# liuzhenboo/Stereo-Visual-Odometry

Measured on AMD Instinct MI355X. Metric: stereo frames/sec on KITTI-00 1241x376; LK-kernel achieved HBM GB/s vs peak, higher is better.
Workload: dtype u8; 1 GPU; S0 synthetic KITTI-like stereo sequence 1241x376 (config #2 stand-in), FAST+LK track_mode LK_stereof2f_pnp, batched frame pairs (256 per step, 4 distinct chunks cycled), frames resident in HBM for `value`; `m1` (--full) = host-resident frames, H2D included; pairs_ok_last_step=256, parallelism=1 GPU

## Files before the change

### include/svo_abi.h

```cpp
#ifndef SVO_ABI_H
#define SVO_ABI_H

#include <stdint.h>

#ifdef __cplusplus
extern "C" {
#endif

#define SVO_ABI_VERSION 9

#define SVO_OK                 0
#define SVO_ERR_ARG           -1
#define SVO_ERR_HIP           -2
#define SVO_ERR_NOMEM         -3
#define SVO_ERR_STATE         -4
#define SVO_FAIL_FEW_KEYPOINTS 1
#define SVO_FAIL_FEW_TRACKS    2
#define SVO_FAIL_INLIER_RATIO  3
#define SVO_FAIL_ROTATION_GATE 4
#define SVO_FAIL_TRANSL_GATE   5
#define SVO_FAIL_CAPACITY      6

#define SVO_MEM_HOST   0
#define SVO_MEM_DEVICE 1
// ... 23 lines not shown
    double  P1[12], P2[12];
    int32_t track_mode;
    int32_t orb_nfeatures;
    float   orb_scale_factor;
    int32_t orb_nlevels;
    int32_t orb_ini_th, orb_min_th;
    int32_t lk_accum;
    int32_t fast_keep_strongest;
} svo_config;

#define SVO_MODE_LK  0
#define SVO_MODE_ORB 1
#define SVO_LK_ACCUM_EXACT 0
#define SVO_LK_ACCUM_SSE2  1
#define SVO_LK_ACCUM_SIMD128 2
#define SVO_LK_ACCUM_SSE2_LEGACY 3

typedef struct {
    double rvec[3], tvec[3], R[9];
    int32_t n_inliers, ransac_iters, best_iter, lm_iters, ok, _pad;
} svo_pnp_result;

typedef struct {
    int32_t ok;
    int32_t fail_stage;
    int32_t n_prev_kps, n_cur_kps, n_tracked, n_inliers;
    int32_t ransac_iters, lm_iters;
    double  rvec[3], tvec[3], R[9];
    double  T_rel_inv[16];
    double  pose[16];
} svo_step_result;

int         svo_abi_version(void);
int         svo_config_bytes(void);
void        svo_default_config(svo_config *cfg, int width, int height);
int         svo_device_count(int *n);
int         svo_create(const svo_config *cfg, int device, svo_ctx **out);
void        svo_destroy(svo_ctx *ctx);
const char *svo_last_error(const svo_ctx *ctx);
int         svo_set_stream(svo_ctx *ctx, void *hip_stream);
int         svo_sync(svo_ctx *ctx);
int         svo_wait_stream(svo_ctx *ctx, void *hip_stream);
int         svo_signal_stream(svo_ctx *ctx, void *hip_stream);
int         svo_signal_stream_inputs(svo_ctx *ctx, void *hip_stream);
int         svo_num_levels(const svo_ctx *ctx);


int svo_fast_detect(svo_ctx *ctx, const uint8_t *img, int pitch, int mem, int threshold,
                    int nonmax, svo_keypoint *out, int cap, int *n_out);

int svo_build_pyramid(svo_ctx *ctx, int slot, const uint8_t *img, int pitch, int mem);
int svo_read_pyramid_level(svo_ctx *ctx, int slot, int level, uint8_t *out, int out_pitch, int mem,
                           int *w, int *h);

int svo_lk_track(svo_ctx *ctx, int slot_prev, int slot_next, const svo_pt2f *prev_pts, int n,
                 svo_pt2f *next_pts, uint8_t *status, int mem);

int svo_circular_match(svo_ctx *ctx, int slot_prevL, int slot_prevR, int slot_curL, int slot_curR,
                       const svo_pt2f *t1_left, int n, svo_pt2f *out_t1_left,
                       svo_pt2f *out_t1_right, svo_pt2f *out_t2_right, svo_pt2f *out_t2_left,
                       int *m_out, int mem);

int svo_triangulate(svo_ctx *ctx, const double P1[12], const double P2[12], const svo_pt2f *x1,
                    const svo_pt2f *x2, int n, svo_pt3f *out, int mem);

int svo_pnp_ransac(svo_ctx *ctx, const svo_pt3f *obj, const svo_pt2f *img, int n, const double K[9],
                   int iterations, float reproj_err, double confidence, svo_pnp_result *res,
                   uint8_t *inlier_mask, int mem);

int svo_orb_extract(svo_ctx *ctx, const uint8_t *img, int pitch, int mem, svo_keypoint *kps, uint8_t *desc,
                    int cap, int *n_out, int *per_level);
int svo_orb_read_level(svo_ctx *ctx, int level, uint8_t *out, int *w, int *h);
int svo_orb_read_candidates(svo_ctx *ctx, int level, float *out4, int cap, int *n_out);

int svo_match_hamming(svo_ctx *ctx, const uint8_t *query, int nq, const uint8_t *train, int nt, int32_t *train_idx,
                      float *distance, int mem);


int svo_add_frame(svo_ctx *ctx, const uint8_t *left, const uint8_t *right, int pitch, int mem,
                  svo_step_result *res);
int svo_reset(svo_ctx *ctx);
int svo_get_pose(svo_ctx *ctx, double pose[16]);
int svo_set_pose(svo_ctx *ctx, const double pose[16]);

int svo_track_batch(svo_ctx *ctx, const uint8_t *left_frames, const uint8_t *right_frames,
                    int pitch, int64_t frame_stride, int n_frames, const double *pose0,
                    svo_step_result *results, int results_mem);

int svo_set_overlap(svo_ctx *ctx, int on);
int svo_wait_results(svo_ctx *ctx);

int svo_host_alloc(svo_ctx *ctx, size_t bytes, void **out);
int svo_host_free(svo_ctx *ctx, void *p);
int svo_upload_frames(svo_ctx *ctx, int buf, const uint8_t *left_frames, const uint8_t *right_frames,
                      int pitch, int64_t frame_stride, int n_frames);
int svo_upload_frames_at(svo_ctx *ctx, int buf, int first_slot, const uint8_t *left_frames, const uint8_t *right_frames,
                         int pitch, int64_t frame_stride, int n_frames);
int svo_wait_upload(svo_ctx *ctx, int buf);
int svo_track_uploaded(svo_ctx *ctx, int buf, int n_frames, const double *pose0,
                       svo_step_result *results, int results_mem);
#define SVO_CONTINUE_CHAIN       1
#define SVO_CONTINUE_CARRY_FRAME 2
int svo_track_uploaded_async(svo_ctx *ctx, int buf, int n_frames, const double *pose0, int continue_chain);
int svo_collect_results(svo_ctx *ctx, svo_step_result *results, int n_pairs);
int svo_results_ready(svo_ctx *ctx, int *n_pairs);

// ... 133 lines not shown
```

### stereo-visual-odometry_amd/binding.py

```python
import ctypes as C
import os
import subprocess

import numpy as np

_HERE = os.path.dirname(os.path.abspath(__file__))
_LIB = None

MEM_HOST, MEM_DEVICE = 0, 1

KP_DTYPE = np.dtype([("x", "<f4"), ("y", "<f4"), ("size", "<f4"), ("angle", "<f4"),
                     ("response", "<f4"), ("octave", "<i4"), ("class_id", "<i4")])


class SvoError(RuntimeError):
    pass


class Config(C.Structure):
    _fields_ = [("width", C.c_int32), ("height", C.c_int32), ("max_keypoints", C.c_int32),
                ("max_batch", C.c_int32), ("num_slots", C.c_int32), ("fast_threshold", C.c_int32),
                ("num_features_tracking", C.c_int32), ("iterations", C.c_int32),
                ("reproj_err", C.c_float), ("confidence", C.c_float),
                ("feature_match_error", C.c_double), ("inlier_rate", C.c_double),
# ... 300 lines not shown
            return
        self.signal_stream(other)

    @property
    def num_levels(self):
        return self.lib.svo_num_levels(self.h)

    def set_overlap(self, on=True):
        self._check(self.lib.svo_set_overlap(self.h, int(on)))

    def wait_results(self):
        self._check(self.lib.svo_wait_results(self.h))

    def enable_timing(self, on=True):
        self._check(self.lib.svo_enable_timing(self.h, int(on)))

    def get_timing(self):
        names = (C.c_char_p * 64)()
        ms = (C.c_float * 64)()
        n = self.lib.svo_get_timing(self.h, names, ms, 64)
        return [(names[i].decode(), float(ms[i])) for i in range(n)]

    def _img(self, img, shape=None):
        shape = shape or (self.height, self.width)
        assert tuple(img.shape) == tuple(shape), (tuple(img.shape), shape)
        if isinstance(img, np.ndarray):
            assert img.dtype == np.uint8 and img.strides[1] == 1
            return C.c_void_p(img.ctypes.data), int(img.strides[0]), MEM_HOST
        assert img.element_size() == 1 and img.stride(1) == 1
        return C.c_void_p(img.data_ptr()), int(img.stride(0)), (MEM_DEVICE if img.is_cuda else MEM_HOST)

    def fast_detect(self, img, threshold=20, nonmax=True, cap=None):
        cap = cap or self.cfg.max_keypoints
        p, pitch, mem = self._img(img)
        out = np.zeros(cap, dtype=KP_DTYPE)
        n = C.c_int(0)
        self._check(self.lib.svo_fast_detect(self.h, p, pitch, mem, int(threshold), int(bool(nonmax)),
                                             C.c_void_p(out.ctypes.data), cap, C.byref(n)))
        return out[:n.value].copy()

    def build_pyramid(self, slot, img):
        p, pitch, mem = self._img(img)
        self._check(self.lib.svo_build_pyramid(self.h, int(slot), p, pitch, mem))

    def read_pyramid_level(self, slot, level):
        w, h = C.c_int(0), C.c_int(0)
        self._check(self.lib.svo_read_pyramid_level(self.h, slot, level, None, 0, MEM_HOST,
                                                    C.byref(w), C.byref(h)))
        out = np.zeros((h.value, w.value), np.uint8)
        self._check(self.lib.svo_read_pyramid_level(self.h, slot, level, C.c_void_p(out.ctypes.data),
                                                    w.value, MEM_HOST, C.byref(w), C.byref(h)))
        return out

    def lk_track(self, slot_prev, slot_next, pts):
        if isinstance(pts, np.ndarray):
            pts = np.ascontiguousarray(pts, np.float32).reshape(-1, 2)
            n = pts.shape[0]
            out = np.zeros((n, 2), np.float32)
            st = np.zeros(n, np.uint8)
        else:
            import torch
            n = pts.shape[0]
            out = torch.zeros((n, 2), dtype=torch.float32, device=pts.device)
            st = torch.zeros(n, dtype=torch.uint8, device=pts.device)
            self._order_in(st)
        pi, mem = _ptr(pts)
        po, _ = _ptr(out)
        ps, _ = _ptr(st)
        self._check(self.lib.svo_lk_track(self.h, slot_prev, slot_next, pi, n, po, ps, mem))
        if mem == MEM_DEVICE:
            self._order_out(st)
        return out, st

    def circular_match(self, slots, t1_left):
        if isinstance(t1_left, np.ndarray):
            t1_left = np.ascontiguousarray(t1_left, np.float32).reshape(-1, 2)
            n = t1_left.shape[0]
            outs = [np.zeros((max(n, 1), 2), np.float32) for _ in range(4)]
        else:
            import torch
            n = t1_left.shape[0]
            outs = [torch.zeros((max(n, 1), 2), dtype=torch.float32, device=t1_left.device) for _ in range(4)]
            self._order_in(outs[0])
        pi, mem = _ptr(t1_left)
        m = C.c_int(0)
        self._check(self.lib.svo_circular_match(self.h, *[int(s) for s in slots], pi, n,
                                                *[_ptr(o)[0] for o in outs], C.byref(m), mem))
        return [o[:m.value] for o in outs]

    def triangulate(self, P1, P2, x1, x2):
        P1 = np.ascontiguousarray(P1, np.float64).reshape(12)
        P2 = np.ascontiguousarray(P2, np.float64).reshape(12)
        if isinstance(x1, np.ndarray):
            x1 = np.ascontiguousarray(x1, np.float32).reshape(-1, 2)
            x2 = np.ascontiguousarray(x2, np.float32).reshape(-1, 2)
            out = np.zeros((x1.shape[0], 3), np.float32)
        else:
            import torch
            out = torch.zeros((x1.shape[0], 3), dtype=torch.float32, device=x1.device)
            self._order_in(out)
        p1, mem = _ptr(x1)
        p2, _ = _ptr(x2)
        self._check(self.lib.svo_triangulate(self.h, C.c_void_p(P1.ctypes.data), C.c_void_p(P2.ctypes.data),
                                             p1, p2, x1.shape[0], _ptr(out)[0], mem))
        if mem == MEM_DEVICE:
            self._order_out(out)
# ... 752 lines not shown
```

### stereo-visual-odometry_amd/csrc/pipeline.hip

```cpp
#include <cstring>
#include "abi_io.h"
#include "carry.h"

namespace svo {

void timing_mark(svo_ctx *ctx, const char *name)
{
    if (!ctx->timing) return;
    if (ctx->ev_used >= 16384) return;
    if (ctx->ev_used == ctx->ev_pool.size()) {
        hipEvent_t ev = nullptr;
        if (dev_event(ctx, &ev, hipEventDefault) != SVO_OK) return;
        ctx->ev_pool.push_back(ev);
    }
    hipEvent_t ev = ctx->ev_pool[ctx->ev_used++];
    (void)hipEventRecord(ev, ctx->stream);
    ctx->marks.emplace_back(name, ev);
}
static inline void mark(svo_ctx *ctx, const char *name) { timing_mark(ctx, name); }

static const char *kTMatch = "orb_match";
static const char *kT0 = "start", *kTPyr = "pyramid", *kTFast = "fast", *kTLk = "lk", *kTCompact = "compact",
                  *kTTri = "triangulate", *kTPnp = "pnp", *kTRefine = "refine", *kTFin = "finalize";

static int ingest_frames(svo_ctx *ctx, const uint8_t *L, const uint8_t *R, int pitch, int64_t frame_stride,
                         int f0, int n_new)
{
    if (ctx->cfg.track_mode == SVO_MODE_ORB) {
        const int rc = orb_extract_batch(ctx, L, R, pitch, frame_stride, 2 * f0, 2 * n_new, ctx->stream,  true);
        if (rc == SVO_OK && ctx->orbm_mode == SVO_ORB_MATCHER_GUIDED) return orbm_stereo_frames(ctx, 2 * f0, n_new, ctx->stream);
        return rc;
    }
    const PyrGeom &g = ctx->geom;
    PyrArgs p{};
    p.g = g; p.pitch = pitch; p.img_stride = frame_stride; p.slot_stride = g.slot_bytes;
    p.img = L; p.img2 = R; p.slots = ctx->bslots + (size_t)(2 * f0) * g.slot_bytes;
    launch_pyramid(p, 2 * n_new, ctx->stream);
    mark(ctx, kTPyr);
    if (ctx->lk_detector == SVO_DETECTOR_GFTT) {
        const int rc = gftt_detect_frames(ctx, L, pitch, frame_stride, f0, n_new);
        mark(ctx, kTFast);
        return rc;
    }
    FastArgs a{};
    a.img = L; a.pitch = pitch; a.img_stride = frame_stride;
    a.w = ctx->cfg.width; a.h = ctx->cfg.height; a.thr = ctx->cfg.fast_threshold; a.nms = 1;
    a.score = ctx->score + (size_t)f0 * ctx->score_stride; a.spitch = ctx->spitch; a.score_stride = ctx->score_stride;
    a.rowcount = ctx->rowcount + (size_t)f0 * ctx->rowcount_stride; a.rowcount_stride = ctx->rowcount_stride;
    a.kp_xy = ctx->kp_xy + (size_t)f0 * ctx->cfg.max_keypoints;
    a.kp_resp = ctx->kp_resp + (size_t)f0 * ctx->cfg.max_keypoints;
    a.kp_stride = ctx->cfg.max_keypoints;
    a.n_out = ctx->kp_n + f0; a.cap = ctx->cfg.max_keypoints;
    launch_fast(a, n_new, ctx->stream);
    if (ctx->bucket_keep > 0) {
        BucketArgs k{};
        k.kp_xy = a.kp_xy; k.kp_resp = a.kp_resp; k.kp_stride = a.kp_stride; k.n_out = a.n_out; k.cap = a.cap;
        k.w = a.w; k.h = a.h; k.cw = ctx->bucket_w; k.ch = ctx->bucket_h; k.per_cell = ctx->bucket_keep;
        k.cols = (a.w + k.cw - 1) / k.cw; k.ncells = k.cols * ((a.h + k.ch - 1) / k.ch);
        k.cells_stride = (int64_t)4 * k.ncells;
        k.cells = ctx->bucket_cells.base ? (int *)ctx->bucket_cells.base + (size_t)f0 * k.cells_stride : nullptr;
        launch_fast_buckets(k, n_new, ctx->stream);
    }
    launch_fast_keep_strongest(a, n_new, ctx->cfg.fast_keep_strongest, ctx->stream);
    mark(ctx, kTFast);
    return SVO_OK;
}

struct StreamStep { const int32_t *ids; const uint8_t *init; };
static int run_back(svo_ctx *ctx, int n_pairs, const double *pose0_host, svo_step_result *results_dev, bool triangulate_first = false,
                    const StreamStep *ss = nullptr);
static const char *kTGather = "stream_gather", *kTScatter = "stream_scatter";

static int stream_segments(svo_ctx *ctx, uint8_t *work[kMaxSeg], size_t bytes[kMaxSeg], int is_count[kMaxSeg])
{
    const size_t cap = (size_t)ctx->cfg.max_keypoints;
    if (ctx->cfg.track_mode == SVO_MODE_ORB) {
        const size_t kcap = (size_t)ctx->orb_kp_cap;
        work[0] = (uint8_t *)ctx->orb_kps;      bytes[0] = 2 * kcap * sizeof(svo_keypoint); is_count[0] = 0;
        work[1] = ctx->orb_desc;                bytes[1] = 2 * kcap * 32;                   is_count[1] = 0;
        work[2] = (uint8_t *)ctx->orb_n;        bytes[2] = 2 * sizeof(int);                 is_count[2] = 1;
        work[3] = (uint8_t *)ctx->orb_overflow; bytes[3] = 2 * sizeof(int);                 is_count[3] = 1;
        if (ctx->orbm_mode == SVO_ORB_MATCHER_GUIDED) {
            work[4] = ctx->orbm_frames;         bytes[4] = ctx->orbm_frame_bytes;           is_count[4] = 0;
            return 5;
        }
    } else {
        work[0] = ctx->bslots;                  bytes[0] = (size_t)2 * ctx->geom.slot_bytes; is_count[0] = 0;
        work[1] = (uint8_t *)ctx->kp_xy;        bytes[1] = cap * sizeof(float2);            is_count[1] = 0;
        work[2] = (uint8_t *)ctx->kp_resp;      bytes[2] = cap * sizeof(float);             is_count[2] = 0;
        work[3] = (uint8_t *)ctx->kp_n;         bytes[3] = sizeof(int);                     is_count[3] = 1;
// ... 482 lines not shown
```

### stereo-visual-odometry_amd/csrc/pyramid.hip

```cpp
#include "svo_device.h"
#include "svo_kernels.h"

namespace svo {

__device__ __forceinline__ const uint8_t *src_image(const PyrArgs &a, int b)
{
    if (a.img2) return ((b & 1) ? a.img2 : a.img) + (int64_t)(b >> 1) * a.img_stride;
    return a.img + (int64_t)b * a.img_stride;
}

__global__ __launch_bounds__(256) void pyr_copy0_kernel(PyrArgs a)
{
    const int b = blockIdx.z, y = blockIdx.y * blockDim.y + threadIdx.y;
    const int w = a.g.w[0];
    if (y >= a.g.h[0]) return;
    const uint8_t *src = src_image(a, b) + (int64_t)y * a.pitch;
    uint8_t *dst = a.slots + (int64_t)b * a.slot_stride + a.g.origin[0] + (int64_t)y * a.g.pitch[0];
    const int x = (blockIdx.x * blockDim.x + threadIdx.x) * 16;
    if (x >= w) return;
    if (x + 16 <= w && ((uintptr_t)(src + x) & 15) == 0) {
        *(uint4 *)(dst + x) = *(const uint4 *)(src + x);
    } else {
        for (int q = 0; q < 16 && x + q < w; q++) dst[x + q] = src[x + q];
    }
}

constexpr int kBorderRows = 16;
constexpr int kFrameRowsPerWg = 4, kSidePasses = 4;
__host__ __device__ inline int border_top_groups() { return 2 * kPad / kFrameRowsPerWg; }
__host__ __device__ inline int border_side_groups(int h) { return (h + kBorderRows * kSidePasses - 1) / (kBorderRows * kSidePasses); }
__global__ __launch_bounds__(256) void pyr_border_kernel(PyrArgs a, int l)
{
    const int b = blockIdx.y;
    const int w = a.g.w[l], h = a.g.h[l], pitch = a.g.pitch[l];
    uint8_t *lvl = a.slots + (int64_t)b * a.slot_stride + a.g.origin[l];
    if ((int)blockIdx.x < border_top_groups()) {
        for (int q = 0; q < kFrameRowsPerWg; q++) {
            const int gidx = blockIdx.x * kFrameRowsPerWg + q;
            const int py = gidx < kPad ? gidx - kPad : h + (gidx - kPad);
            const uint8_t *src = lvl + (int64_t)refl101(py, h) * pitch;
            uint8_t *dst = lvl + (int64_t)py * pitch;
            for (int px = ((int)threadIdx.x << 2) - kPad; px < w + kPad; px += 1024) {
                uint32_t v = 0;
                if (px >= 0 && px + 4 <= w) v = *(const uint32_t *)(src + px);
                else {
#pragma unroll
                    for (int k = 0; k < 4; k++) v |= (uint32_t)src[refl101(min(px + k, w + kPad - 1), w)] << (8 * k);
                }
                if (px + 4 <= w + kPad) *(uint32_t *)(dst + px) = v;
                else for (int k = 0; px + k < w + kPad; k++) dst[px + k] = (uint8_t)(v >> (8 * k));
            }
        }
        return;
    }
    const int sgroup = blockIdx.x - border_top_groups();
    if (w >= 2 * kPad) {
        static_assert(kBorderRows == 16 && kPad == 32, "256 threads = 16 rows x 16 dwords");
        typedef uint32_t u32_unaligned __attribute__((aligned(1)));
        const int k = threadIdx.x & 15, r = threadIdx.x >> 4;
        const int px = k < 8 ? -kPad + 4 * k : w + 4 * (k - 8);
        const int c0 = k < 8 ? kPad - 3 - 4 * k : w - 5 - 4 * (k - 8);
        for (int q = 0; q < kSidePasses; q++) {
            const int py = (sgroup * kSidePasses + q) * kBorderRows + r;
            if (py >= h) return;
            uint8_t *row = lvl + (int64_t)py * pitch;
            const uint32_t v = *(const u32_unaligned *)(row + c0);
            *(u32_unaligned *)(row + px) = __builtin_amdgcn_perm(0u, v, 0x00010203u);
        }
    } else {
        const int t = threadIdx.x & 63;
        const int px = t < kPad ? t - kPad : w + (t - kPad);
        const int sx = refl101(px, w);
        for (int q = 0; q < kSidePasses; q++)
            for (int r = threadIdx.x >> 6; r < kBorderRows; r += 4) {
                const int py = (sgroup * kSidePasses + q) * kBorderRows + r;
                if (py >= h) return;
                uint8_t *row = lvl + (int64_t)py * pitch;
                row[px] = row[sx];
            }
    }
}

__global__ __launch_bounds__(256) void pyr_down_kernel(PyrArgs a, int l)
{
    const int b = blockIdx.z, y = blockIdx.y * blockDim.y + threadIdx.y;
    const int w = a.g.w[l];
    if (y >= a.g.h[l]) return;
    const int sp = a.g.pitch[l - 1];
    uint8_t *slot = a.slots + (int64_t)b * a.slot_stride;
    const uint8_t *src = slot + a.g.origin[l - 1];
    uint8_t *dst = slot + a.g.origin[l] + (int64_t)y * a.g.pitch[l];
    const int x0 = (blockIdx.x * blockDim.x + threadIdx.x) * 4;
    if (x0 >= w) return;
    int acc[4] = {0, 0, 0, 0};
#pragma unroll
    for (int r = 0; r < 5; r++) {
        const uint32_t *row = (const uint32_t *)(src + (int64_t)(2 * y + r - 2) * sp + 2 * x0 - 4);
        const uint32_t d0 = row[0], d1 = row[1], d2 = row[2], d3 = row[3];
        int s[16];
#pragma unroll
        for (int j = 0; j < 4; j++) {
            s[j] = (d0 >> (8 * j)) & 255; s[4 + j] = (d1 >> (8 * j)) & 255;
            s[8 + j] = (d2 >> (8 * j)) & 255; s[12 + j] = (d3 >> (8 * j)) & 255;
        }
        const int wv = (r == 2) ? 6 : ((r == 1 || r == 3) ? 4 : 1);
#pragma unroll
        for (int q = 0; q < 4; q++) {
            const int c = 4 + 2 * q;
            const int hs = s[c] * 6 + (s[c - 1] + s[c + 1]) * 4 + s[c - 2] + s[c + 2];
            acc[q] += hs * wv;
        }
    }
    uint32_t out = 0;
#pragma unroll
    for (int q = 0; q < 4; q++) out |= (uint32_t)((acc[q] + 128) >> 8) << (8 * q);
    if (x0 + 4 <= w) *(uint32_t *)(dst + x0) = out;
    else for (int q = 0; x0 + q < w; q++) dst[x0 + q] = (uint8_t)(out >> (8 * q));
}

__global__ __launch_bounds__(256) void pyr_read_level_kernel(PyrGeom g, const uint8_t *slot, int l,
                                                              uint8_t *out, int out_pitch)
{
    int x = blockIdx.x * 256 + threadIdx.x, y = blockIdx.y;
    if (x >= g.w[l]) return;
    out[(int64_t)y * out_pitch + x] = slot[g.origin[l] + (int64_t)y * g.pitch[l] + x];
}

void launch_pyramid(const PyrArgs &a, int batch, hipStream_t st)
{
    dim3 blk(256, 1, 1);
    auto shape = [](int lanes_per_row, int rows, dim3 &grid, dim3 &block, int batch) {
        const int bx = lanes_per_row < 256 ? lanes_per_row : 256, by = 256 / bx;
        block = dim3(bx, by, 1);
        grid = dim3((lanes_per_row + bx - 1) / bx, (rows + by - 1) / by, batch);
    };
    {
        dim3 g, bk;
        shape((a.g.w[0] + 15) / 16, a.g.h[0], g, bk, batch);
        hipLaunchKernelGGL(pyr_copy0_kernel, g, bk, 0, st, a);
    }
    for (int l = 0; l < a.g.nlevels; l++) {
        if (l > 0) {
            dim3 g, bk;
            shape((a.g.w[l] + 3) / 4, a.g.h[l], g, bk, batch);
            hipLaunchKernelGGL(pyr_down_kernel, g, bk, 0, st, a, l);
        }
        dim3 gb(border_top_groups() + border_side_groups(a.g.h[l]), batch, 1);
        hipLaunchKernelGGL(pyr_border_kernel, gb, blk, 0, st, a, l);
    }
}

void launch_pyr_read_level(const PyrGeom &g, const uint8_t *slot, int l, uint8_t *out, int out_pitch,
                           hipStream_t st)
{
    dim3 grid((g.w[l] + 255) / 256, g.h[l], 1), blk(256, 1, 1);
    hipLaunchKernelGGL(pyr_read_level_kernel, grid, blk, 0, st, g, slot, l, out, out_pitch);
}

}
```

### stereo-visual-odometry_amd/csrc/svo_abi.hip

```cpp
#include <algorithm>
#include <cmath>
#include <cstdio>
#include <cstring>
#include <ctime>
#include <new>
#include <vector>
#include "abi_io.h"
#include "carry.h"
#include "fast_scratch.h"

using namespace svo;

namespace svo {
int dev_alloc_raw(svo_ctx *ctx, void **out, size_t bytes)
{
    *out = nullptr;
    if (bytes == 0) bytes = 1;
    if (ctx->arena.planning) {
        ctx->arena.plan.emplace_back(out, ctx->arena.planned);
        ctx->arena.planned += align_up(bytes, kDevAlign);
        return SVO_OK;
    }
    SVO_HIP(hipMalloc(out, bytes));
    ctx->arena.extra.push_back(*out);
    return SVO_OK;
}

int dev_defer(svo_ctx *ctx, std::function<int()> fn)
{
    if (!ctx->arena.planning) return fn();
    ctx->arena.after.push_back(std::move(fn));
    return SVO_OK;
}

static int dev_commit(svo_ctx *ctx)
{
    DevArena &a = ctx->arena;
    a.planning = false;
    SVO_HIP(hipMalloc((void **)&a.base, a.planned + 256));
    for (auto &e : a.plan) *e.first = a.base + e.second;
    a.plan.clear();
    for (auto &fn : a.after) { const int rc = fn(); if (rc != SVO_OK) return rc; }
    a.after.clear();
    return SVO_OK;
}

int dev_reserve(svo_ctx *ctx, DevScratch *s, size_t bytes)
{
    if (s->base && bytes <= s->bytes) return SVO_OK;
    uint8_t *grown = nullptr;
    SVO_HIP(hipMalloc((void **)&grown, bytes ? bytes : 1));
    uint8_t *old = s->base;
    if (!old) ctx->arena.scratch.push_back(s);
    s->base = grown; s->bytes = bytes;
    if (old) (void)hipFree(old);
    return SVO_OK;
}

int dev_event(svo_ctx *ctx, hipEvent_t *ev, unsigned flags)
{
    if (*ev) return SVO_OK;
    SVO_HIP(hipEventCreateWithFlags(ev, flags));
// ... 100 lines not shown
    DevArena &a = c->arena;
    for (hipEvent_t e : a.events) (void)hipEventDestroy(e);
    for (size_t k = a.streams.size(); k-- > 0;) (void)hipStreamDestroy(a.streams[k]);
    a.events.clear(); a.streams.clear();
}

static double now_ms()
{
    timespec ts;
    clock_gettime(CLOCK_MONOTONIC, &ts);
    return ts.tv_sec * 1e3 + ts.tv_nsec * 1e-6;
}
#define PHASE(name) do { if (timing_on) { const double t__ = now_ms(); fprintf(stderr, "[svo_create] %8.2f ms  %s\n", t__ - t_phase, name); t_phase = t__; } } while (0)

extern "C" int svo_create(const svo_config *cfg, int device, svo_ctx **out)
{
    if (!cfg || !out) return SVO_ERR_ARG;
    const bool timing_on = getenv("SVO_TIMING") != nullptr;
    double t_phase = now_ms();
    *out = nullptr;
    if (cfg->width < 32 || cfg->height < 32 || cfg->max_keypoints < 64 || cfg->max_batch < 1 ||
        cfg->num_slots < 4 || cfg->width > kMaxFrameSide || cfg->height > kMaxFrameSide)
        return SVO_ERR_ARG;
    if (cfg->lk_accum != SVO_LK_ACCUM_EXACT && cfg->lk_accum != SVO_LK_ACCUM_SSE2 && cfg->lk_accum != SVO_LK_ACCUM_SIMD128 &&
        cfg->lk_accum != SVO_LK_ACCUM_SSE2_LEGACY) {
        fprintf(stderr, "svo_create: lk_accum = %d is none of SVO_LK_ACCUM_EXACT / _SSE2 / _SIMD128 / _SSE2_LEGACY\n", cfg->lk_accum);
        return SVO_ERR_ARG;
    }
    if (cfg->fast_keep_strongest < 0) return SVO_ERR_ARG;
    if (cfg->num_features_tracking < 4) {
        fprintf(stderr, "svo_create: num_features_tracking = %d < 4 is not supported (cv::solvePnPRansac asserts npoints >= 4)\n",
                cfg->num_features_tracking);
        return SVO_ERR_ARG;
    }
    svo_ctx *ctx = new (std::nothrow) svo_ctx();
    if (!ctx) return SVO_ERR_NOMEM;
    ctx->cfg = *cfg;
    ctx->device = device;
    for (int i = 0; i < 16; i++) ctx->pose[i] = (i % 5 == 0) ? 1.0 : 0.0;
    int ndev = 0;
    if (hipGetDeviceCount(&ndev) != hipSuccess || ndev <= 0 || device < 0 || device >= ndev) {
        fprintf(stderr, "svo_create: no usable HIP device (count=%d, requested %d)\n", ndev, device);
        delete ctx;
        return SVO_ERR_HIP;
    }
    PHASE("hipGetDeviceCount (HIP runtime start)");
    auto fail = [&](int code) { free_all(ctx); delete ctx; return code; };
#define CK(call) do { if ((call) != 0) { fprintf(stderr, "svo_create: %s failed\n", #call); return fail(SVO_ERR_HIP); } } while (0)
    CK(hipSetDevice(device));
    CK(dev_stream(ctx, &ctx->own_stream));
    ctx->stream = ctx->own_stream;
    PHASE("hipSetDevice + stream");
    make_geom(cfg->width, cfg->height, &ctx->geom);

    const int w = cfg->width, h = cfg->height, cap = cfg->max_keypoints, B = cfg->max_batch;
    const int n_img = B + 1;
    ctx->n_img = n_img;
    const bool orb = cfg->track_mode == SVO_MODE_ORB;
    if (!orb && cfg->track_mode != SVO_MODE_LK) return fail(SVO_ERR_ARG);
    const int n_fast = orb ? 1 : n_img, B_lk = orb ? 1 : B;
    ctx->arena.planning = true;
#define DA(ptr, bytes) do { if (dev_alloc(ctx, &(ptr), (bytes)) != SVO_OK) return fail(SVO_ERR_HIP); } while (0)
    DA(ctx->slots, (size_t)cfg->num_slots * ctx->geom.slot_bytes);
    dev_defer(ctx, [ctx]() { SVO_HIP(hipMemsetAsync(ctx->slots, 0, (size_t)ctx->cfg.num_slots * ctx->geom.slot_bytes, ctx->stream)); return SVO_OK; });
    ctx->slot_built.assign(cfg->num_slots, 0);
    ctx->stage_pitch = align_up(w, 256);
    DA(ctx->stage_img, (size_t)ctx->stage_pitch * h * 2);
    ctx->spitch = fast_record_pitch(w);
    ctx->score_stride = (int64_t)ctx->spitch * h;
    DA(ctx->score, (size_t)ctx->score_stride * n_fast);
    ctx->rowcount_stride = fast_count_words(w, h);
    DA(ctx->rowcount, sizeof(int) * (size_t)ctx->rowcount_stride * n_fast);
    DA(ctx->kp_xy, sizeof(float2) * (size_t)cap * n_fast);
    DA(ctx->kp_resp, sizeof(float) * (size_t)cap * n_fast);
    DA(ctx->kp_n, sizeof(int) * (size_t)n_fast);
    DA(ctx->pts_in, sizeof(float2) * (size_t)cap * B_lk);
    for (int i = 0; i < 4; i++) {
        DA(ctx->pts_out[i], sizeof(float2) * (size_t)cap * B_lk);
        DA(ctx->status[i], (size_t)cap * B_lk);
        DA(ctx->cmp[i], sizeof(float2) * (size_t)cap * B);
    }
    DA(ctx->keep, (size_t)cap * B_lk);
    DA(ctx->m_out, sizeof(int) * (size_t)B);
    DA(ctx->X3, sizeof(float) * 3 * (size_t)cap * B);
    if (geom_workspace_bytes(*cfg, B, &ctx->pnp_ws_bytes) != SVO_OK) return fail(SVO_ERR_ARG);
    PHASE("plan + kernel attributes (code object load)");
    DA(ctx->pnp_ws, ctx->pnp_ws_bytes);
    dev_defer(ctx, [ctx]() { return geom_workspace_init(ctx); });
    DA(ctx->d_results, sizeof(svo_step_result) * (size_t)B);
    DA(ctx->bslots, orb ? 256 : (size_t)2 * n_img * ctx->geom.slot_bytes);
    DA(ctx->kp_n_snap, sizeof(int) * (size_t)(3 * n_img));
    if (B > 1) {
        const size_t per_cam = (size_t)ctx->stage_pitch * h * (size_t)(B + 1);
        for (int k = 0; k < 2; k++) {
            DA(ctx->fb[k], 2 * per_cam);
            DA(ctx->d_async[k], sizeof(svo_step_result) * (size_t)B);
        }
    }
    if (orb) {
        int rc = orb_alloc(ctx);
        if (rc != SVO_OK) { fprintf(stderr, "svo_create: %s\n", ctx->err.c_str()); return fail(rc); }
    }
#undef DA
    if (dev_commit(ctx) != SVO_OK) { fprintf(stderr, "svo_create: device memory (%zu MB): %s\n", ctx->arena.planned >> 20, ctx->err.c_str()); return fail(SVO_ERR_HIP); }
    PHASE("one device allocation + deferred initialisation");
    CK(hipHostMalloc(&ctx->h_stage, (size_t)ctx->stage_pitch * h * 2, hipHostMallocDefault));
// ... 146 lines not shown
    SVO_ARG(pitch >= ctx->cfg.width, "pitch < width");
    if (mem == SVO_MEM_DEVICE) { *dptr = img; *dpitch = pitch; return SVO_OK; }
    SVO_ARG(mem == SVO_MEM_HOST, "mem must be SVO_MEM_HOST or SVO_MEM_DEVICE");
    return svo::stage_host_image(ctx, img, pitch, stage_idx, dptr, dpitch);
}

extern "C" int svo_fast_detect(svo_ctx *ctx, const uint8_t *img, int pitch, int mem, int threshold,
                               int nonmax, svo_keypoint *out, int cap, int *n_out)
{
    if (!ctx) return SVO_ERR_ARG;
    SVO_ARG(out && n_out && cap >= 0, "null output");
    SVO_HIP(hipSetDevice(ctx->device));
    const uint8_t *d; int dp;
    int rc = resolve_image(ctx, img, pitch, mem, 0, &d, &dp);
    if (rc) return rc;
    FastArgs a{};
    a.img = d; a.pitch = dp; a.img_stride = 0;
    a.w = ctx->cfg.width; a.h = ctx->cfg.height;
    a.thr = threshold < 0 ? 0 : (threshold > 255 ? 255 : threshold);
    a.nms = nonmax != 0;
    a.score = ctx->score; a.spitch = ctx->spitch; a.score_stride = ctx->score_stride;
    a.rowcount = ctx->rowcount; a.rowcount_stride = ctx->rowcount_stride;
    a.kp_xy = ctx->kp_xy; a.kp_resp = ctx->kp_resp; a.kp_stride = ctx->cfg.max_keypoints;
    a.n_out = ctx->kp_n; a.cap = ctx->cfg.max_keypoints;
    launch_fast(a, 1, ctx->stream);
    SVO_HIP(hipGetLastError());
    int n;
    SVO_TRY(count_read(ctx, ctx->kp_n, &n));
    *n_out = n;
    if (n > ctx->cfg.max_keypoints) { ctx->err = "FAST: keypoints exceed max_keypoints"; return SVO_ERR_ARG; }
    if (n > cap) { ctx->err = "FAST: keypoints exceed caller capacity"; return SVO_ERR_ARG; }
    if (n == 0) return SVO_OK;
    float2 *h_xy;
    SVO_TRY(pinned_block(ctx, (sizeof(float2) + sizeof(float)) * (size_t)ctx->cfg.max_keypoints, &h_xy));
    float *h_r = (float *)(h_xy + ctx->cfg.max_keypoints);
    SVO_TRY(from_device(ctx, h_xy, (const float2 *)ctx->kp_xy, (size_t)n, SVO_MEM_HOST));
    SVO_TRY(from_device(ctx, h_r, (const float *)ctx->kp_resp, (size_t)n, SVO_MEM_HOST));
    SVO_TRY(io_done(ctx, SVO_MEM_HOST));
    format_keypoints(h_xy, h_r, n, out);
    return SVO_OK;
}

extern "C" int svo_build_pyramid(svo_ctx *ctx, int slot, const uint8_t *img, int pitch, int mem)
{
    if (!ctx) return SVO_ERR_ARG;
    SVO_ARG(slot >= 0 && slot < ctx->cfg.num_slots, "slot out of range");
    SVO_HIP(hipSetDevice(ctx->device));
    const uint8_t *d; int dp;
    int rc = resolve_image(ctx, img, pitch, mem, 0, &d, &dp);
    if (rc) return rc;
    PyrArgs a{};
    a.g = ctx->geom; a.img = d; a.pitch = dp; a.img_stride = 0;
    a.slots = ctx->slots + (size_t)slot * ctx->geom.slot_bytes; a.slot_stride = 0;
    launch_pyramid(a, 1, ctx->stream);
    SVO_HIP(hipGetLastError());
    if (mem == SVO_MEM_HOST) SVO_HIP(hipStreamSynchronize(ctx->stream));
    ctx->slot_built[slot] = 1;
    return SVO_OK;
}

extern "C" int svo_read_pyramid_level(svo_ctx *ctx, int slot, int level, uint8_t *out, int out_pitch,
                                      int mem, int *w, int *h)
{
    if (!ctx) return SVO_ERR_ARG;
    SVO_ARG(slot >= 0 && slot < ctx->cfg.num_slots, "slot out of range");
    SVO_ARG(level >= 0 && level < ctx->geom.nlevels, "level out of range");
    if (!ctx->slot_built[slot]) { ctx->err = "pyramid slot not built"; return SVO_ERR_STATE; }
    const int lw = ctx->geom.w[level], lh = ctx->geom.h[level];
    if (w) *w = lw;
    if (h) *h = lh;
    if (!out) return SVO_OK;
    SVO_ARG(out_pitch >= lw, "out_pitch < level width");
    SVO_HIP(hipSetDevice(ctx->device));
    const uint8_t *s = ctx->slots + (size_t)slot * ctx->geom.slot_bytes;
    if (mem == SVO_MEM_DEVICE) {
        launch_pyr_read_level(ctx->geom, s, level, out, out_pitch, ctx->stream);
        SVO_HIP(hipGetLastError());
        return SVO_OK;
    }
    SVO_HIP(hipMemcpy2DAsync(out, out_pitch, s + ctx->geom.origin[level], ctx->geom.pitch[level], lw, lh,
                             hipMemcpyDeviceToHost, ctx->stream));
    SVO_HIP(hipStreamSynchronize(ctx->stream));
    return SVO_OK;
}

static void fill_lk_common(svo_ctx *ctx, LkArgs &a, int n)
{
    a.g = ctx->geom;
    a.slot_stride = 0;
    a.pts_stride = 0;
    a.n_pts = nullptr; a.n_fixed = n; a.cap = n;
    a.match_err = ctx->cfg.feature_match_error;
    a.accum = ctx->cfg.lk_accum;
}

extern "C" int svo_lk_track(svo_ctx *ctx, int slot_prev, int slot_next, const svo_pt2f *prev_pts, int n,
                            svo_pt2f *next_pts, uint8_t *status, int mem)
{
    if (!ctx) return SVO_ERR_ARG;
    SVO_ARG(slot_prev >= 0 && slot_prev < ctx->cfg.num_slots && slot_next >= 0 &&
            slot_next < ctx->cfg.num_slots, "slot out of range");
    SVO_ARG(n >= 0 && n <= ctx->cfg.max_keypoints, "n exceeds max_keypoints");
    SVO_ARG(mem == SVO_MEM_HOST || mem == SVO_MEM_DEVICE, "bad mem");
    if (!ctx->slot_built[slot_prev] || !ctx->slot_built[slot_next]) { ctx->err = "pyramid slot not built"; return SVO_ERR_STATE; }
    if (n == 0) return SVO_OK;
    SVO_ARG(prev_pts && next_pts && status, "null pointer");
    SVO_HIP(hipSetDevice(ctx->device));
    const float2 *d_in;
    SVO_TRY(to_device(ctx, (const float2 *)prev_pts, ctx->pts_in, (size_t)n, mem, &d_in));
    LkArgs a{};
    fill_lk_common(ctx, a, n);
    a.ncalls = 1;
    a.prev[0] = ctx->slots + (size_t)slot_prev * ctx->geom.slot_bytes;
    a.next[0] = ctx->slots + (size_t)slot_next * ctx->geom.slot_bytes;
    a.pts_in = d_in;
    a.pts_out[0] = mem == SVO_MEM_DEVICE ? (float2 *)next_pts : ctx->pts_out[0];
    a.status[0] = mem == SVO_MEM_DEVICE ? status : ctx->status[0];
    launch_lk(a, 1, n, ctx->stream);
    SVO_HIP(hipGetLastError());
    SVO_TRY(from_device(ctx, (float2 *)next_pts, (const float2 *)a.pts_out[0], (size_t)n, mem));
    SVO_TRY(from_device(ctx, status, (const uint8_t *)a.status[0], (size_t)n, mem));
    return io_done(ctx, mem);
}

extern "C" int svo_circular_match(svo_ctx *ctx, int slot_prevL, int slot_prevR, int slot_curL, int slot_curR,
                                  const svo_pt2f *t1_left, int n, svo_pt2f *out_t1_left,
                                  svo_pt2f *out_t1_right, svo_pt2f *out_t2_right, svo_pt2f *out_t2_left,
                                  int *m_out, int mem)
{
    if (!ctx) return SVO_ERR_ARG;
    const int sl[4] = {slot_prevL, slot_prevR, slot_curL, slot_curR};
    for (int i = 0; i < 4; i++) {
        SVO_ARG(sl[i] >= 0 && sl[i] < ctx->cfg.num_slots, "slot out of range");
        if (!ctx->slot_built[sl[i]]) { ctx->err = "pyramid slot not built"; return SVO_ERR_STATE; }
    }
// ... 1279 lines not shown
```

### stereo-visual-odometry_amd/csrc/svo_ctx.h

```cpp
#pragma once
#include <hip/hip_runtime.h>
#include <functional>
#include <string>
#include <utility>
#include <vector>
#include "../../include/svo_abi.h"
#include "block_cut.h"
#include "pinned_layout.h"
#include "svo_kernels.h"

struct DevScratch {
    uint8_t *base = nullptr;
    size_t bytes = 0;
};

struct DevArena {
    char *base = nullptr;
    size_t planned = 0;
    bool planning = false;
    std::vector<std::pair<void **, size_t>> plan;
    std::vector<std::function<int()>> after;
    std::vector<void *> extra;
    std::vector<DevScratch *> scratch;
    std::vector<hipEvent_t> events;
// ... 5 lines not shown
    int n = 0;
    int n_seg = 0;
    uint8_t *seg[kMaxSeg] = {};
    size_t seg_bytes[kMaxSeg] = {};
    double *pose = nullptr;
    long long *next_id = nullptr;
    std::vector<uint8_t> has_ids, restart;
    std::vector<int> n_frames;
    std::vector<int> seen;
    int call = 0;
};

struct ResizeShape {
    int bx_shift = 8, rpt = 8;
    int lds_pitch = 0, lds_rows = 0;
};

struct ResizeTab {
    int sw = 0, sh = 0, dw = 0, dh = 0, interp = 0;
    double fx = 0, fy = 0;
    double inv_x = 1, inv_y = 1;
    bool box = false;
    void *xt = nullptr, *yt = nullptr;
    ResizeShape shape;
};

struct Ingest {
    bool on = false;
    int sw = 0, sh = 0, tab = -1;
    int spitch = 0;
    uint8_t *work = nullptr;
    DevScratch src_stage;
    uint8_t *up_stage[2] = {nullptr, nullptr};
};

struct GfttBuf : DevScratch {
    float *map = nullptr; int mpitch = 0; int64_t map_stride = 0;
    unsigned *maxkey = nullptr; int *n_cand = nullptr;
    unsigned long long *keys = nullptr; int64_t keys_stride = 0;
    int *cells = nullptr; int64_t cells_stride = 0;
};

struct svo_ctx {
    svo_config cfg;
    DevArena arena;
    int device = 0;
    hipStream_t own_stream = nullptr, stream = nullptr;
    std::string err;
    svo::PyrGeom geom;

    int n_img = 0;
    uint8_t *slots = nullptr;
    std::vector<char> slot_built;
    uint8_t *stage_img = nullptr;
    int stage_pitch = 0;
    uint8_t *h_stage = nullptr;
    hipEvent_t ev_stage[2] = {nullptr, nullptr};
    bool h_stage_busy[2] = {false, false};
    uint8_t *score = nullptr; int spitch = 0; int64_t score_stride = 0;
    int *rowcount = nullptr; int64_t rowcount_stride = 0;
    float2 *kp_xy = nullptr; float *kp_resp = nullptr; int *kp_n = nullptr;
    float2 *pts_in = nullptr;
    float2 *pts_out[4] = {nullptr, nullptr, nullptr, nullptr};
    uint8_t *status[4] = {nullptr, nullptr, nullptr, nullptr};
    uint8_t *keep = nullptr;
    float2 *cmp[4] = {nullptr, nullptr, nullptr, nullptr};
    int *m_out = nullptr;
    float *X3 = nullptr;
    void *pnp_ws = nullptr; size_t pnp_ws_bytes = 0;
    svo_step_result *d_results = nullptr;
    uint8_t *bslots = nullptr;
    int online_frames = 0;
    int online_cur = 0;
    int last_batch_pairs = 0;
    int carry_slot = -1;
    int online_tracked = 0;
    double pose[16];
    bool orb_ready = false;
    bool orb_qt_parallel = false;
    bool orb_level0_in_slot = false;
    bool orb_resize_staged = false;
    ResizeShape orb_resize_shape[svo::kOrbMaxLevels];
    bool orb_copy_level0 = false;
    svo::OrbGeom orb_geom;
    uint8_t *orb_slots = nullptr, *orb_blur = nullptr;
    void *orb_xtab = nullptr, *orb_ytab = nullptr;
    float4 *orb_cell_cand = nullptr; int *orb_cell_cnt = nullptr;
    float4 *orb_lvl_cand = nullptr; int *orb_lvl_cnt = nullptr;
    int orb_node_cap = 0;
    void *orb_qkeys = nullptr, *orb_qtmp = nullptr;
    int *orb_sel = nullptr, *orb_sel_cnt = nullptr, *orb_overflow = nullptr;
    void *orb_kps = nullptr; uint8_t *orb_desc = nullptr; int *orb_n = nullptr; int orb_kp_cap = 0, orb_cand_cap = 0;
    int *orb_midx[2] = {nullptr, nullptr}; float *orb_mdist[2] = {nullptr, nullptr};
    int orbm_mode = SVO_ORB_MATCHER_BRUTE, orbm_th_stereo = 75, orbm_th_track = 100;
    double orbm_ratio = 0.9, orbm_radius = 0.0, orbm_max_disparity = 0.0;
    int orbm_epoch = 0;
    int orbm_kc = 0; size_t orbm_frame_bytes = 0;
    uint8_t *orbm_frames = nullptr;
    float2 *orbm_t2 = nullptr; int *orbm_mj = nullptr; unsigned *orbm_mkey = nullptr, *orbm_win = nullptr;
    svo::OrbL0 orb_l0{}; int orb_l0_slot0 = 0;
    void *h_pinned = nullptr; svo::PinnedLayout pinned;
    bool overlap = false;
    hipStream_t side_stream = nullptr;
    uint8_t *fb[2] = {nullptr, nullptr};
    hipStream_t copy_stream = nullptr;
    hipEvent_t ev_up[2] = {nullptr, nullptr}, ev_fb_free[2] = {nullptr, nullptr};
// ... 162 lines not shown
```

Before: 19850 stereo pairs/s.

## Fuse pyramid border padding into level copy and downsample kernels

Each pyramid level used to be built by one kernel, and a second kernel then filled the reflected border. Now the copy or downsample kernel writes the mirrored border rows and columns itself: extra lanes handle the side pads and each row is also stored to its reflected top or bottom row. This halves the launches per level and avoids re-reading the level to fill its padding. It adds unaligned and duplicate stores, an SVO_PYR_LEGACY fallback, and debug accessors for reading the padded frame and counting routes.

```diff
diff --git a/include/svo_abi.h b/include/svo_abi.h
--- a/include/svo_abi.h
+++ b/include/svo_abi.h
@@ -99,6 +99,9 @@
 int svo_build_pyramid(svo_ctx *ctx, int slot, const uint8_t *img, int pitch, int mem);
 int svo_read_pyramid_level(svo_ctx *ctx, int slot, int level, uint8_t *out, int out_pitch, int mem,
                            int *w, int *h);
+int svo_read_pyramid_frame(svo_ctx *ctx, int slot, int level, uint8_t *out, int out_pitch, int mem,
+                           int *w, int *h);
+int svo_pyramid_routes(const svo_ctx *ctx, long long *levels_framed, long long *levels_border);
 
 int svo_lk_track(svo_ctx *ctx, int slot_prev, int slot_next, const svo_pt2f *prev_pts, int n,
                  svo_pt2f *next_pts, uint8_t *status, int mem);
diff --git a/stereo-visual-odometry_amd/binding.py b/stereo-visual-odometry_amd/binding.py
--- a/stereo-visual-odometry_amd/binding.py
+++ b/stereo-visual-odometry_amd/binding.py
@@ -376,6 +376,20 @@
                                                     w.value, MEM_HOST, C.byref(w), C.byref(h)))
         return out
 
+    def read_pyramid_frame(self, slot, level):
+        w, h = C.c_int(0), C.c_int(0)
+        self._check(self.lib.svo_read_pyramid_frame(self.h, slot, level, None, 0, MEM_HOST,
+                                                    C.byref(w), C.byref(h)))
+        out = np.zeros((h.value, w.value), np.uint8)
+        self._check(self.lib.svo_read_pyramid_frame(self.h, slot, level, C.c_void_p(out.ctypes.data),
+                                                    w.value, MEM_HOST, C.byref(w), C.byref(h)))
+        return out
+
+    def pyramid_routes(self):
+        framed, border = C.c_longlong(0), C.c_longlong(0)
+        self._check(self.lib.svo_pyramid_routes(self.h, C.byref(framed), C.byref(border)))
+        return framed.value, border.value
+
     def lk_track(self, slot_prev, slot_next, pts):
         if isinstance(pts, np.ndarray):
             pts = np.ascontiguousarray(pts, np.float32).reshape(-1, 2)
diff --git a/stereo-visual-odometry_amd/csrc/pipeline.hip b/stereo-visual-odometry_amd/csrc/pipeline.hip
--- a/stereo-visual-odometry_amd/csrc/pipeline.hip
+++ b/stereo-visual-odometry_amd/csrc/pipeline.hip
@@ -1,6 +1,7 @@
 #include <cstring>
 #include "abi_io.h"
 #include "carry.h"
+#include "pyr_frames.h"
 
 namespace svo {
 
@@ -35,7 +36,7 @@
     PyrArgs p{};
     p.g = g; p.pitch = pitch; p.img_stride = frame_stride; p.slot_stride = g.slot_bytes;
     p.img = L; p.img2 = R; p.slots = ctx->bslots + (size_t)(2 * f0) * g.slot_bytes;
-    launch_pyramid(p, 2 * n_new, ctx->stream);
+    build_pyramids(ctx, p, 2 * n_new, ctx->stream);
     mark(ctx, kTPyr);
     if (ctx->lk_detector == SVO_DETECTOR_GFTT) {
         const int rc = gftt_detect_frames(ctx, L, pitch, frame_stride, f0, n_new);
diff --git a/stereo-visual-odometry_amd/csrc/pyr_frames.h b/stereo-visual-odometry_amd/csrc/pyr_frames.h
--- /dev/null
+++ b/stereo-visual-odometry_amd/csrc/pyr_frames.h
@@ -0,0 +1,21 @@
+#pragma once
+#include "svo_ctx.h"
+
+namespace svo {
+
+inline bool pyr_level_framed(const PyrGeom &g, int l) { return g.w[l] >= kPad + 1 && g.h[l] >= kPad + 1; }
+
+void launch_pyramid_legacy(const PyrArgs &a, int batch, hipStream_t st);
+void launch_pyr_read_frame(const PyrGeom &g, const uint8_t *slot, int l, uint8_t *out, int out_pitch, hipStream_t st);
+
+inline void build_pyramids(svo_ctx *ctx, const PyrArgs &a, int batch, hipStream_t st)
+{
+    for (int l = 0; l < a.g.nlevels; l++) {
+        if (!ctx->pyr_legacy && pyr_level_framed(a.g, l)) ctx->pyr_levels_framed++;
+        else ctx->pyr_levels_border++;
+    }
+    if (ctx->pyr_legacy) launch_pyramid_legacy(a, batch, st);
+    else launch_pyramid(a, batch, st);
+}
+
+}
diff --git a/stereo-visual-odometry_amd/csrc/pyramid.hip b/stereo-visual-odometry_amd/csrc/pyramid.hip
--- a/stereo-visual-odometry_amd/csrc/pyramid.hip
+++ b/stereo-visual-odometry_amd/csrc/pyramid.hip
@@ -1,5 +1,6 @@
 #include "svo_device.h"
 #include "svo_kernels.h"
+#include "pyr_frames.h"
 
 namespace svo {
 
@@ -81,6 +82,37 @@
     }
 }
 
+__device__ __forceinline__ uint32_t pyr_down4(const uint8_t *p, int sp, bool shift0)
+{
+    int acc[4] = {0, 0, 0, 0};
+#pragma unroll
+    for (int r = 0; r < 5; r++) {
+        const uint32_t *row = (const uint32_t *)(p + (int64_t)r * sp);
+        uint32_t d0 = row[0], d1 = row[1], d2 = row[2], d3 = row[3];
+        if (shift0) {
+            d3 = __builtin_amdgcn_alignbit(d3, d2, 16); d2 = __builtin_amdgcn_alignbit(d2, d1, 16);
+            d1 = __builtin_amdgcn_alignbit(d1, d0, 16); d0 <<= 16;
+        }
+        int s[16];
+#pragma unroll
+        for (int j = 0; j < 4; j++) {
+            s[j] = (d0 >> (8 * j)) & 255; s[4 + j] = (d1 >> (8 * j)) & 255;
+            s[8 + j] = (d2 >> (8 * j)) & 255; s[12 + j] = (d3 >> (8 * j)) & 255;
+        }
+        const int wv = (r == 2) ? 6 : ((r == 1 || r == 3) ? 4 : 1);
+#pragma unroll
+        for (int q = 0; q < 4; q++) {
+            const int c = 4 + 2 * q;
+            const int hs = s[c] * 6 + (s[c - 1] + s[c + 1]) * 4 + s[c - 2] + s[c + 2];
+            acc[q] += hs * wv;
+        }
+    }
+    uint32_t out = 0;
+#pragma unroll
+    for (int q = 0; q < 4; q++) out |= (uint32_t)((acc[q] + 128) >> 8) << (8 * q);
+    return out;
+}
+
 __global__ __launch_bounds__(256) void pyr_down_kernel(PyrArgs a, int l)
 {
     const int b = blockIdx.z, y = blockIdx.y * blockDim.y + threadIdx.y;
@@ -92,30 +124,82 @@
     uint8_t *dst = slot + a.g.origin[l] + (int64_t)y * a.g.pitch[l];
     const int x0 = (blockIdx.x * blockDim.x + threadIdx.x) * 4;
     if (x0 >= w) return;
-    int acc[4] = {0, 0, 0, 0};
-#pragma unroll
-    for (int r = 0; r < 5; r++) {
-        const uint32_t *row = (const uint32_t *)(src + (int64_t)(2 * y + r - 2) * sp + 2 * x0 - 4);
-        const uint32_t d0 = row[0], d1 = row[1], d2 = row[2], d3 = row[3];
-        int s[16];
-#pragma unroll
-        for (int j = 0; j < 4; j++) {
-            s[j] = (d0 >> (8 * j)) & 255; s[4 + j] = (d1 >> (8 * j)) & 255;
-            s[8 + j] = (d2 >> (8 * j)) & 255; s[12 + j] = (d3 >> (8 * j)) & 255;
-        }
-        const int wv = (r == 2) ? 6 : ((r == 1 || r == 3) ? 4 : 1);
-#pragma unroll
-        for (int q = 0; q < 4; q++) {
-            const int c = 4 + 2 * q;
-            const int hs = s[c] * 6 + (s[c - 1] + s[c + 1]) * 4 + s[c - 2] + s[c + 2];
-            acc[q] += hs * wv;
-        }
-    }
-    uint32_t out = 0;
-#pragma unroll
-    for (int q = 0; q < 4; q++) out |= (uint32_t)((acc[q] + 128) >> 8) << (8 * q);
+    const uint32_t out = pyr_down4(src + (int64_t)(2 * y - 2) * sp + 2 * x0 - 4, sp, false);
     if (x0 + 4 <= w) *(uint32_t *)(dst + x0) = out;
     else for (int q = 0; x0 + q < w; q++) dst[x0 + q] = (uint8_t)(out >> (8 * q));
+}
+
+struct RowCopies { int64_t top, bot; };
+__device__ __forceinline__ RowCopies row_copies(int y, int h, int pitch)
+{
+    RowCopies c;
+    c.top = (y >= 1 && y <= kPad) ? -2 * (int64_t)y * pitch : 0;
+    c.bot = (y >= h - 1 - kPad && y <= h - 2) ? 2 * (int64_t)(h - 1 - y) * pitch : 0;
+    return c;
+}
+typedef uint32_t u32_unaligned __attribute__((aligned(1)));
+template <typename T> __device__ __forceinline__ void store_rows(uint8_t *p, const T &v, const RowCopies &c)
+{
+    *(T *)p = v;
+    if (c.top) *(T *)(p + c.top) = v;
+    if (c.bot) *(T *)(p + c.bot) = v;
+}
+__device__ __forceinline__ uint32_t reverse_bytes(uint32_t v) { return __builtin_amdgcn_perm(0u, v, 0x00010203u); }
+
+constexpr int kFrame0Lanes = 2 * kPad / 16;
+__global__ __launch_bounds__(256) void pyr_frame0_kernel(PyrArgs a)
+{
+    const int b = blockIdx.z, y = blockIdx.y * blockDim.y + threadIdx.y;
+    const int w = a.g.w[0], h = a.g.h[0], pitch = a.g.pitch[0];
+    if (y >= h) return;
+    const uint8_t *src = src_image(a, b) + (int64_t)y * a.pitch;
+    uint8_t *dst = a.slots + (int64_t)b * a.slot_stride + a.g.origin[0] + (int64_t)y * pitch;
+    const RowCopies rc = row_copies(y, h, pitch);
+    const int lane = blockIdx.x * blockDim.x + threadIdx.x, nint = (w + 15) >> 4;
+    if (lane < nint) {
+        const int x = lane * 16;
+        if (x + 16 <= w && ((uintptr_t)(src + x) & 15) == 0) {
+            store_rows(dst + x, *(const uint4 *)(src + x), rc);
+        } else {
+            for (int q = 0; q < 16 && x + q < w; q++) store_rows(dst + x + q, src[x + q], rc);
+        }
+        return;
+    }
+    const int k = lane - nint;
+    if (k >= kFrame0Lanes) return;
+    const int px = k < kFrame0Lanes / 2 ? -kPad + 16 * k : w + 16 * (k - kFrame0Lanes / 2);
+    const int c = k < kFrame0Lanes / 2 ? -px : 2 * (w - 1) - px;
+    uint32_t v[4];
+#pragma unroll
+    for (int i = 0; i < 4; i++) v[i] = reverse_bytes(*(const u32_unaligned *)(src + c - 4 * i - 3));
+#pragma unroll
+    for (int i = 0; i < 4; i++) store_rows<u32_unaligned>(dst + px + 4 * i, v[i], rc);
+}
+
+constexpr int kDownFrameLanes = 2 * kPad / 4;
+__global__ __launch_bounds__(256) void pyr_down_frame_kernel(PyrArgs a, int l)
+{
+    const int b = blockIdx.z, y = blockIdx.y * blockDim.y + threadIdx.y;
+    const int w = a.g.w[l], h = a.g.h[l], pitch = a.g.pitch[l], sp = a.g.pitch[l - 1];
+    if (y >= h) return;
+    uint8_t *slot = a.slots + (int64_t)b * a.slot_stride;
+    const uint8_t *src = slot + a.g.origin[l - 1] + (int64_t)(2 * y - 2) * sp;
+    uint8_t *dst = slot + a.g.origin[l] + (int64_t)y * pitch;
+    const int lane = blockIdx.x * blockDim.x + threadIdx.x, k = lane - ((w + 3) >> 2);
+    if (k >= kDownFrameLanes) return;
+    const bool side = k >= 0;
+    int x0 = lane * 4, px = x0;
+    if (side) {
+        px = k < 8 ? -kPad + 4 * k : w + 4 * (k - 8);
+        x0 = k < 8 ? kPad - 3 - 4 * k : w - 5 - 4 * (k - 8);
+    }
+    const int c0 = 2 * x0 - 2, sh = c0 & 3;
+    const uint32_t out = __builtin_amdgcn_ballot_w64(sh == 0) ? pyr_down4(src + (c0 - sh), sp, sh == 0)
+                                                              : pyr_down4(src + (c0 - sh), sp, false);
+    const RowCopies rc = row_copies(y, h, pitch);
+    if (side) store_rows<u32_unaligned>(dst + px, reverse_bytes(out), rc);
+    else if (x0 + 4 <= w) store_rows(dst + x0, out, rc);
+    else for (int q = 0; x0 + q < w; q++) store_rows(dst + x0 + q, (uint8_t)(out >> (8 * q)), rc);
 }
 
 __global__ __launch_bounds__(256) void pyr_read_level_kernel(PyrGeom g, const uint8_t *slot, int l,
@@ -126,27 +210,52 @@
     out[(int64_t)y * out_pitch + x] = slot[g.origin[l] + (int64_t)y * g.pitch[l] + x];
 }
 
+__global__ __launch_bounds__(256) void pyr_read_frame_kernel(PyrGeom g, const uint8_t *slot, int l,
+                                                              uint8_t *out, int out_pitch)
+{
+    int x = blockIdx.x * 256 + threadIdx.x, y = blockIdx.y;
+    if (x >= g.w[l] + 2 * kPad) return;
+    out[(int64_t)y * out_pitch + x] = slot[g.origin[l] + (int64_t)(y - kPad) * g.pitch[l] + (x - kPad)];
+}
+
+static void pyr_shape(int lanes_per_row, int rows, dim3 &grid, dim3 &block, int batch)
+{
+    const int bx = lanes_per_row < 256 ? lanes_per_row : 256, by = 256 / bx;
+    block = dim3(bx, by, 1);
+    grid = dim3((lanes_per_row + bx - 1) / bx, (rows + by - 1) / by, batch);
+}
+
+static void launch_level_legacy(const PyrArgs &a, int l, int batch, hipStream_t st)
+{
+    dim3 g, bk;
+    if (l == 0) {
+        pyr_shape((a.g.w[0] + 15) / 16, a.g.h[0], g, bk, batch);
+        hipLaunchKernelGGL(pyr_copy0_kernel, g, bk, 0, st, a);
+    } else {
+        pyr_shape((a.g.w[l] + 3) / 4, a.g.h[l], g, bk, batch);
+        hipLaunchKernelGGL(pyr_down_kernel, g, bk, 0, st, a, l);
+    }
+    dim3 gb(border_top_groups() + border_side_groups(a.g.h[l]), batch, 1);
+    hipLaunchKernelGGL(pyr_border_kernel, gb, dim3(256, 1, 1), 0, st, a, l);
+}
+
+void launch_pyramid_legacy(const PyrArgs &a, int batch, hipStream_t st)
+{
+    for (int l = 0; l < a.g.nlevels; l++) launch_level_legacy(a, l, batch, st);
+}
+
 void launch_pyramid(const PyrArgs &a, int batch, hipStream_t st)
 {
-    dim3 blk(256, 1, 1);
-    auto shape = [](int lanes_per_row, int rows, dim3 &grid, dim3 &block, int batch) {
-        const int bx = lanes_per_row < 256 ? lanes_per_row : 256, by = 256 / bx;
-        block = dim3(bx, by, 1);
-        grid = dim3((lanes_per_row + bx - 1) / bx, (rows + by - 1) / by, batch);
-    };
-    {
+    for (int l = 0; l < a.g.nlevels; l++) {
+        if (!pyr_level_framed(a.g, l)) { launch_level_legacy(a, l, batch, st); continue; }
         dim3 g, bk;
-        shape((a.g.w[0] + 15) / 16, a.g.h[0], g, bk, batch);
-        hipLaunchKernelGGL(pyr_copy0_kernel, g, bk, 0, st, a);
-    }
-    for (int l = 0; l < a.g.nlevels; l++) {
-        if (l > 0) {
-            dim3 g, bk;
-            shape((a.g.w[l] + 3) / 4, a.g.h[l], g, bk, batch);
-            hipLaunchKernelGGL(pyr_down_kernel, g, bk, 0, st, a, l);
-        }
-        dim3 gb(border_top_groups() + border_side_groups(a.g.h[l]), batch, 1);
-        hipLaunchKernelGGL(pyr_border_kernel, gb, blk, 0, st, a, l);
+        if (l == 0) {
+            pyr_shape((a.g.w[0] + 15) / 16 + kFrame0Lanes, a.g.h[0], g, bk, batch);
+            hipLaunchKernelGGL(pyr_frame0_kernel, g, bk, 0, st, a);
+        } else {
+            pyr_shape((a.g.w[l] + 3) / 4 + kDownFrameLanes, a.g.h[l], g, bk, batch);
+            hipLaunchKernelGGL(pyr_down_frame_kernel, g, bk, 0, st, a, l);
+        }
     }
 }
 
@@ -157,4 +266,11 @@
     hipLaunchKernelGGL(pyr_read_level_kernel, grid, blk, 0, st, g, slot, l, out, out_pitch);
 }
 
-}
+void launch_pyr_read_frame(const PyrGeom &g, const uint8_t *slot, int l, uint8_t *out, int out_pitch,
+                           hipStream_t st)
+{
+    dim3 grid((g.w[l] + 2 * kPad + 255) / 256, g.h[l] + 2 * kPad, 1), blk(256, 1, 1);
+    hipLaunchKernelGGL(pyr_read_frame_kernel, grid, blk, 0, st, g, slot, l, out, out_pitch);
+}
+
+}
diff --git a/stereo-visual-odometry_amd/csrc/svo_abi.hip b/stereo-visual-odometry_amd/csrc/svo_abi.hip
--- a/stereo-visual-odometry_amd/csrc/svo_abi.hip
+++ b/stereo-visual-odometry_amd/csrc/svo_abi.hip
@@ -8,6 +8,7 @@
 #include "abi_io.h"
 #include "carry.h"
 #include "fast_scratch.h"
+#include "pyr_frames.h"
 
 using namespace svo;
 
@@ -214,6 +215,7 @@
     ctx->stream = ctx->own_stream;
     PHASE("hipSetDevice + stream");
     make_geom(cfg->width, cfg->height, &ctx->geom);
+    { const char *e = getenv("SVO_PYR_LEGACY"); ctx->pyr_legacy = e && e[0] == '1'; }
 
     const int w = cfg->width, h = cfg->height, cap = cfg->max_keypoints, B = cfg->max_batch;
     const int n_img = B + 1;
@@ -466,7 +468,7 @@
     PyrArgs a{};
     a.g = ctx->geom; a.img = d; a.pitch = dp; a.img_stride = 0;
     a.slots = ctx->slots + (size_t)slot * ctx->geom.slot_bytes; a.slot_stride = 0;
-    launch_pyramid(a, 1, ctx->stream);
+    build_pyramids(ctx, a, 1, ctx->stream);
     SVO_HIP(hipGetLastError());
     if (mem == SVO_MEM_HOST) SVO_HIP(hipStreamSynchronize(ctx->stream));
     ctx->slot_built[slot] = 1;
@@ -495,6 +497,40 @@
     SVO_HIP(hipMemcpy2DAsync(out, out_pitch, s + ctx->geom.origin[level], ctx->geom.pitch[level], lw, lh,
                              hipMemcpyDeviceToHost, ctx->stream));
     SVO_HIP(hipStreamSynchronize(ctx->stream));
+    return SVO_OK;
+}
+
+extern "C" int svo_read_pyramid_frame(svo_ctx *ctx, int slot, int level, uint8_t *out, int out_pitch,
+                                      int mem, int *w, int *h)
+{
+    if (!ctx) return SVO_ERR_ARG;
+    SVO_ARG(slot >= 0 && slot < ctx->cfg.num_slots, "slot out of range");
+    SVO_ARG(level >= 0 && level < ctx->geom.nlevels, "level out of range");
+    if (!ctx->slot_built[slot]) { ctx->err = "pyramid slot not built"; return SVO_ERR_STATE; }
+    const int fw = ctx->geom.w[level] + 2 * kPad, fh = ctx->geom.h[level] + 2 * kPad;
+    if (w) *w = fw;
+    if (h) *h = fh;
+    if (!out) return SVO_OK;
+    SVO_ARG(out_pitch >= fw, "out_pitch < padded level width");
+    SVO_HIP(hipSetDevice(ctx->device));
+    const uint8_t *s = ctx->slots + (size_t)slot * ctx->geom.slot_bytes;
+    if (mem == SVO_MEM_DEVICE) {
+        launch_pyr_read_frame(ctx->geom, s, level, out, out_pitch, ctx->stream);
+        SVO_HIP(hipGetLastError());
+        return SVO_OK;
+    }
+    const int pitch = ctx->geom.pitch[level];
+    SVO_HIP(hipMemcpy2DAsync(out, out_pitch, s + ctx->geom.origin[level] - (int64_t)kPad * pitch - kPad, pitch, fw, fh,
+                             hipMemcpyDeviceToHost, ctx->stream));
+    SVO_HIP(hipStreamSynchronize(ctx->stream));
+    return SVO_OK;
+}
+
+extern "C" int svo_pyramid_routes(const svo_ctx *ctx, long long *levels_framed, long long *levels_border)
+{
+    if (!ctx) return SVO_ERR_ARG;
+    if (levels_framed) *levels_framed = ctx->pyr_levels_framed;
+    if (levels_border) *levels_border = ctx->pyr_levels_border;
     return SVO_OK;
 }
 
diff --git a/stereo-visual-odometry_amd/csrc/svo_ctx.h b/stereo-visual-odometry_amd/csrc/svo_ctx.h
--- a/stereo-visual-odometry_amd/csrc/svo_ctx.h
+++ b/stereo-visual-odometry_amd/csrc/svo_ctx.h
@@ -81,6 +81,8 @@
     int n_img = 0;
     uint8_t *slots = nullptr;
     std::vector<char> slot_built;
+    bool pyr_legacy = false;
+    long long pyr_levels_framed = 0, pyr_levels_border = 0;
     uint8_t *stage_img = nullptr;
     int stage_pitch = 0;
     uint8_t *h_stage = nullptr;
```

Result: no change. 19900 stereo pairs/s, median of 6 (+0.3%).
